# nii-yamagishilab/NELE-GAN

Measured on AMD Instinct MI355X. Metric: utterances/sec per GAN_epoch step (G+D+metric loss), higher is better.
Workload: dtype bf16

## Files before the change

### nele_gan_amd/csrc/haspi.hip

```cpp
#include "common.h"
#include <type_traits>
#include <cstdlib>

#define HP_NCH 32
#define HP_FS 24000.0
#define HP_LEVEL 65.0
#define HP_NBASIS 6
#define HP_NMOD 10
#define HP_NWIN 32769
#define HP_NTAB 512
#define HP_SPACE 9
#define HP_NFILT 52
#define HP_NHALF 26

typedef float hp_env_t;

struct HaspiWs {
    double* win;
    float* r24;
    double* mid;
    hp_env_t* ctl;
    hp_env_t* env;
    double* bw;
    double* loss;
    double* ssp;
// ... 8 lines not shown
    int fmul;
    double* benv;
    double* bkt;
    int* shift;
    double* lp;
    int* act;
    int* grank;
    int* gcnt;
    double* cpsum;
    double* cmean;
    int ngb;
    int* info;
    double* cep;
    double* cm;
    double* xf;
    double* cpart;
    const int* lens;
    float* cphi;
    double* sse;
    int fs_in;
    int n24, nsub;
    int nlp, lp_raw;
    int n24p;
};

__device__ __forceinline__ int hp_len(const HaspiWs& ws, int b, int L) { return ws.lens ? min(ws.lens[b], L) : L; }
__host__ __device__ static inline int hp_n24_of(int L, int fs_in) { return fs_in == 24000 ? L : (int)ceil((double)L * (24000.0 / (double)fs_in)); }
__host__ __device__ static inline int hp_nres_of(int L, int fs_in) { return fs_in == 24000 ? L : (int)((double)L * (24000.0 / (double)fs_in)); }
__device__ __forceinline__ int hp_n24(const HaspiWs& ws, int b) {
    if (!ws.lens) return ws.n24;
    return min(ws.n24, hp_n24_of(ws.lens[b], ws.fs_in));
}
__device__ __forceinline__ int hp_nsub(const HaspiWs& ws, int b) { return (hp_n24(ws, b) + HP_SPACE - 1) / HP_SPACE; }
__device__ __forceinline__ int hp_row(int idx, int sig0, int nsig) { return nsig == 2 ? idx : 2 * idx + sig0; }

__device__ __forceinline__ int hp_lp_di(const HaspiWs& ws, int b, int ch) {
    if (!ws.lp_raw) return 0;
    const int sh = ws.shift[(size_t)b * HP_NCH + ch];
    const int ul = (((26 - sh) % 9) + 9) % 9;
    return (ul + sh - 26) / 9;
}
__device__ __forceinline__ double hp_lp_at(const double* __restrict__ lpb, int i, int ch, int di) {
    const int g = i - di;
    return g >= 0 ? lpb[(size_t)g * HP_NCH + ch] : 0.0;
}

// ... 457 lines not shown
        }
        if (part == 0) {
#pragma unroll
            for (int u = 0; u < HP_CH; ++u) out[(size_t)(n0 + u) * HP_NCH] = (hp_env_t)eo[u];
        }
    }
    return ss;
}

#define GS_RC 16
#define GS_LC 1536
#define GS_MAXC 160
__device__ __forceinline__ void hp_rotate(double& cold, double& sold, double cn, double sn) {
    const double arg = fma(sold, sn, cold * cn);
    sold = fma(sold, cn, -(cold * sn));
    cold = arg;
}
__device__ __forceinline__ void hp_gt_step(const GtCoef& c, double x, double y, double& r0, double& r1, double& r2, double& r3) {
    r0 = fma(c.a1, x + y, r1);
    r1 = fma(c.a5, x, fma(c.a2, y, r2));
    r2 = fma(c.a3, y, r3);
    r3 = c.a4 * y;
}
__global__ __launch_bounds__(128) void haspi_pmat_kernel(HaspiWs ws, int lc, int signal, int sig0, int nsig) {
    const int ch = threadIdx.x & 31, k = threadIdx.x >> 5;
    const int row = signal ? hp_row(blockIdx.x, sig0, nsig) : 0;
    const double BW = signal ? ws.bw[(size_t)row * HP_NCH + ch] : hp_bw1(ch);
    const GtCoef c = hp_gt(BW, hp_cfreq(ch));
    double r0 = (k == 0), r1 = (k == 1), r2 = (k == 2), r3 = (k == 3);
    for (int n = 0; n < lc; ++n) {
        const double yr = r0;
        r0 = c.a1 * yr + r1;
        r1 = c.a2 * yr + r2;
        r2 = c.a3 * yr + r3;
        r3 = c.a4 * yr;
    }
    double* P = ws.pmat + ((size_t)(signal ? 1 + row : 0) * HP_NCH + ch) * 16;
    P[0 * 4 + k] = r0; P[1 * 4 + k] = r1; P[2 * 4 + k] = r2; P[3 * 4 + k] = r3;
}

template <bool SIGNAL>
__global__ __launch_bounds__(64) void haspi_bank_prefix_kernel(HaspiWs ws, int sig0, int nsig) {
    const int row = hp_row(blockIdx.x, sig0, nsig), lane = threadIdx.x, ch = lane & 31;
    const int n24 = hp_n24(ws, row >> 1);
    const int nch = ((n24 + GS_RC - 1) / GS_RC * GS_RC + ws.lc - 1) / ws.lc;
    const double* P = ws.pmat + ((size_t)(SIGNAL ? 1 + row : 0) * HP_NCH + ch) * 16;
    double Pm[16];
#pragma unroll
    for (int q = 0; q < 16; ++q) Pm[q] = P[q];
    double* est = ws.est + (size_t)row * ws.nchunk * 256 + lane;
    double r0 = 0, r1 = 0, r2 = 0, r3 = 0;
    constexpr int G = 8;
    for (int j0 = 0; j0 < nch; j0 += G) {
        double e[G][4];
#pragma unroll
        for (int g = 0; g < G; ++g) {
            const int j = min(j0 + g, nch - 1);
#pragma unroll
            for (int q = 0; q < 4; ++q) e[g][q] = est[(size_t)j * 256 + 64 * q];
        }
#pragma unroll
        for (int g = 0; g < G; ++g) {
            if (j0 + g < nch) {
                double* o = est + (size_t)(j0 + g) * 256;
                o[0] = r0; o[64] = r1; o[128] = r2; o[192] = r3;
                const double t0 = ((Pm[0] * r0 + Pm[1] * r1) + (Pm[2] * r2 + Pm[3] * r3)) + e[g][0];
                const double t1 = ((Pm[4] * r0 + Pm[5] * r1) + (Pm[6] * r2 + Pm[7] * r3)) + e[g][1];
                const double t2 = ((Pm[8] * r0 + Pm[9] * r1) + (Pm[10] * r2 + Pm[11] * r3)) + e[g][2];
                const double t3 = ((Pm[12] * r0 + Pm[13] * r1) + (Pm[14] * r2 + Pm[15] * r3)) + e[g][3];
// ... 10 lines not shown
__device__ __forceinline__ float hp_exp2f(float x) { return __builtin_amdgcn_exp2f(x); }
struct IhcC { double R2, R12C1, R23C2, a11, a12, a21, a22, denom, R1inv, c10, c11, c12, c20, c21, c22; };
__device__ __forceinline__ IhcC hp_ihc_consts() {
    const double delta = 2.0;
    const double tau1 = 0.001 * 2, tau2 = 0.001 * 60;
    const double T = 1 / HP_FS;
    const double R1 = 1 / delta, R2 = 0.5 * (1 - R1), R3 = R2;
    const double C1 = tau1 * (R1 + R2) / (R1 * R2);
    const double C2 = tau2 / ((R1 + R2) * R3);
    IhcC k;
    k.a11 = R1 + R2 + R1 * R2 * (C1 / T); k.a12 = -R1; k.a21 = -R3; k.a22 = R2 + R3 + R2 * R3 * (C2 / T);
    k.denom = 1.0 / (k.a11 * k.a22 - k.a21 * k.a12);
    k.R1inv = 1.0 / R1; k.R12C1 = R1 * R2 * (C1 / T); k.R23C2 = R2 * R3 * (C2 / T); k.R2 = R2;
    k.c10 = k.denom * k.a22 * k.R2;  k.c11 = k.denom * k.a22 * k.R12C1;  k.c12 = -k.denom * k.a12 * k.R23C2;
    k.c20 = -k.denom * k.a21 * k.R2; k.c21 = -k.denom * k.a21 * k.R12C1; k.c22 = k.denom * k.a11 * k.R23C2;
    return k;
}
__device__ __forceinline__ void hp_ihc_step(const IhcC& k, double V0, double& V1, double& V2) {
    const double t1 = fma(k.c12, V2, fma(k.c11, V1, V0 * k.c10));
    const double t2 = fma(k.c22, V2, fma(k.c21, V1, V0 * k.c20));
    V1 = t1; V2 = t2;
}

template <bool SIGNAL, bool PASS2, bool BM = false, bool GAIN = false>
__global__ __launch_bounds__(64) void haspi_bank_scan_kernel(HaspiWs ws, int sig0) {
    const int b = blockIdx.z, sig = sig0 + blockIdx.y, lane = threadIdx.x, ch = lane & 31;
    const int chunk = 2 * blockIdx.x + (lane >> 5);
    const int row = 2 * b + sig, lc = ws.lc;
    const int n24 = hp_n24(ws, b);
    const int n0 = chunk * lc, n1 = min(n0 + lc, (n24 + GS_RC - 1) / GS_RC * GS_RC);
    if (n0 >= n1) return;
    const double cf = hp_cfreq(ch);
    const GtCoef c = hp_gt(SIGNAL ? ws.bw[(size_t)row * HP_NCH + ch] : hp_bw1(ch), cf);
    const double tpt = 2.0 * M_PI / HP_FS;
    const double cn = cos(tpt * cf), sn = sin(tpt * cf);
    double* est = ws.est + ((size_t)row * ws.nchunk + chunk) * 256 + ch;
    double r0 = 0, r1 = 0, r2 = 0, r3 = 0, i0 = 0, i1 = 0, i2 = 0, i3 = 0;
    if (PASS2) {
        r0 = est[0]; r1 = est[64]; r2 = est[128]; r3 = est[192];
        i0 = est[32]; i1 = est[96]; i2 = est[160]; i3 = est[224];
    }
    double cold, sold;
    {
        const double ang = tpt * cf * (double)(n0 - 1);
        cold = cos(ang);
        sold = -sin(ang);
    }
// ... 8 lines not shown
    const double gb0 = 0.095107983402496, ga1 = -0.809784033195007;
    const IhcC ik = hp_ihc_consts();
    float knee = 30.0f, attn = 0.f;
    if (GAIN) {
        const HpLoss ls = hp_loss(ws, sig, ch);
        slope = (float)(1.0 - (1.0 / ls.CR));
        knee = (float)ls.lowknee; attn = (float)ls.attnOHC;
        c_off = (float)(HP_LEVEL + 20.0 * log10(hp_gt(hp_bw1(ch), cf).gain));
        s_off = (float)(HP_LEVEL - ls.attnIHC + 20.0 * log10(c.gain));
        for (int n = max(0, n0 - GL_W); n < n0; n += GL_U) {
            float gc[GL_U];
#pragma unroll
            for (int u = 0; u < GL_U; ++u) gc[u] = ctl[(size_t)(n + u) * HP_NCH];
#pragma unroll
            for (int u = 0; u < GL_U; ++u) {
                float le = c_off + TEN_LOG10_2 * hp_log2f(gc[u]);
                le = fminf(fmaxf(le, knee), 100.0f);
                const double gx = (double)hp_exp2f((-attn - (le - knee) * slope) * LOG2_10_OVER_20);
                const double y = gb0 * gx + gz;
                gz = gb0 * gx - ga1 * y;
            }
        }
    }
    for (int nb = n0; nb < n1; nb += GS_RC) {
        double xc[GS_RC];
        const hp_env_t* ctl_nb = ctl + (size_t)nb * HP_NCH;
        hp_env_t* out_nb = out + (size_t)nb * HP_NCH;
        float* cph_nb = BM ? cph + (size_t)nb * HP_NCH : nullptr;
#pragma unroll
        for (int u = 0; u < GS_RC / 2; ++u) {
            const double2 v = *reinterpret_cast<const double2*>(xin + nb + 2 * u);
            xc[2 * u] = v.x; xc[2 * u + 1] = v.y;
        }
        float eo[GS_RC], co[BM ? GS_RC : 1];
        auto bank = [&](auto tail_tag) {
            constexpr bool TAIL = decltype(tail_tag)::value;
#pragma unroll
            for (int u = 0; u < GS_RC; ++u) {
                hp_rotate(cold, sold, cn, sn);
                const double xr = xc[u] * cold, xi = xc[u] * sold;
                const double yr = xr + r0, yi = xi + i0;
                hp_gt_step(c, xr, yr, r0, r1, r2, r3);
                hp_gt_step(c, xi, yi, i0, i1, i2, i3);
                if (PASS2) {
                    const double e2 = yr * yr + yi * yi;
                    eo[u] = (float)e2;
                    if (!SIGNAL || BM) ss += (!TAIL || nb + u < n24) ? e2 : 0.0;
                    if (BM) co[u] = e2 > 0.0 ? (float)((yr * cold + yi * sold) / sqrt(e2)) : 0.f;
                }
            }
        };
        if (PASS2 && (!SIGNAL || BM) && nb + GS_RC > n24) bank(std::true_type{}); else bank(std::false_type{});
        if (GAIN) {
            float gc[GS_RC];
#pragma unroll
            for (int u = 0; u < GS_RC; ++u) gc[u] = ctl_nb[u * HP_NCH];
#pragma unroll
            for (int u = 0; u < GS_RC; ++u) {
                float le = c_off + TEN_LOG10_2 * hp_log2f(gc[u]);
                le = fminf(fmaxf(le, knee), 100.0f);
                const double gx = (double)hp_exp2f((-attn - (le - knee) * slope) * LOG2_10_OVER_20);
                const double yl = gb0 * gx + gz;
                gz = gb0 * gx - ga1 * yl;
                const float g = (float)yl;
                float y = s_off + TEN_LOG10_2 * hp_log2f(g * g * eo[u]);
                y = y > 0.0f ? y : 0.0f;
                eo[u] = y;
                hp_ihc_step(ik, (double)y, V1, V2);
            }
        }
        if (PASS2) {
#pragma unroll
            for (int u = 0; u < GS_RC; ++u) out_nb[u * HP_NCH] = eo[u];
            if (BM) {
#pragma unroll
                for (int u = 0; u < GS_RC; ++u) cph_nb[u * HP_NCH] = co[u];
            }
        }
    }
    if (!PASS2) {
        est[0] = r0; est[64] = r1; est[128] = r2; est[192] = r3;
        est[32] = i0; est[96] = i1; est[160] = i2; est[224] = i3;
    } else if (!SIGNAL) {
        ws.ssp[((size_t)row * ws.nchunk + chunk) * HP_NCH + ch] = ss;
    } else if (BM) {
        ws.sse[((size_t)row * ws.nchunk + chunk) * HP_NCH + ch] = ss;
    }
    if (GAIN) {
        const int ncg = (ws.n24p + ws.lcg - 1) / ws.lcg;
        double* ihe = ws.ihe + ((size_t)row * ncg + chunk) * 64 + ch;
        ihe[0] = V1; ihe[32] = V2;
    }
}

template <bool SIGNAL>
__global__ __launch_bounds__(512) void haspi_bank_tail_kernel(HaspiWs ws, int sig0, int nsig, int full, int nrows) {
    __shared__ double stage[2][64][GS_RC + 1];
    __shared__ int wred[8];
    const int id = (int)blockIdx.x, slot = id >> 3, cgrp = slot & 3, rest = slot >> 2;
    const int ncg = (ws.nchunk + 63) / 64;
    const int ridx = (rest / ncg) * 8 + (id & 7);
    if (ridx >= nrows) return;
    const int row = hp_row(ridx, sig0, nsig), b = row >> 1;
    const int tid = threadIdx.x, lane = tid & 63, wv = tid >> 6, ch = 8 * cgrp + wv;
    const int c0 = 64 * (rest % ncg), chunk = c0 + lane, lc = ws.lc;
    const int n24 = hp_n24(ws, b), nend = (n24 + GS_RC - 1) / GS_RC * GS_RC;
    const int n0 = chunk * lc, n1 = min(n0 + lc, nend);
    const bool live = n0 < n1;
    const double cf = hp_cfreq(ch);
    const double BW = SIGNAL ? ws.bw[(size_t)row * HP_NCH + ch] : hp_bw1(ch);
    const GtCoef c = hp_gt(BW, cf);
    const double tpt = 2.0 * M_PI / HP_FS;
    int W;
    {
        const double la = BW * tpt * (24.7 + cf / 9.26449) * 1.019;
        const double npk = fmax(3.0 / la, 1.0);
        const double peak = 3.0 * log(npk) - la * npk;
        double nn = 60.0 / la;
// ... 3 lines not shown
        if (full == 1) W = lc;
        if (full == 2) W = GS_RC;
    }
    if (lane == 0) wred[wv] = W;
    __syncthreads();
    int Wmax = wred[0];
#pragma unroll
    for (int q = 1; q < 8; ++q) Wmax = max(Wmax, wred[q]);
    const double cn = cos(tpt * cf), sn = sin(tpt * cf);
    double cold, sold;
    {
        const double ang = tpt * cf * (double)(n1 - W - 1);
        cold = cos(ang);
        sold = -sin(ang);
    }
    const double* xin = ws.mid + (size_t)row * ws.n24p;
    const int cc = tid >> 3, part = tid & 7;
    const int cn0 = (c0 + cc) * lc, cn1 = min(cn0 + lc, nend);
    const double* psrc = xin + (cn1 - Wmax + 2 * part);
    const int pfirst = (cn0 < cn1) ? cn0 - (cn1 - Wmax + 2 * part) : 0x7fffffff;
    double2 pv = (0 >= pfirst) ? *reinterpret_cast<const double2*>(psrc) : make_double2(0.0, 0.0);
    double r0 = 0, r1 = 0, r2 = 0, r3 = 0, i0 = 0, i1 = 0, i2 = 0, i3 = 0;
    const int tjoin = Wmax - W;
    for (int t = 0, it = 0; t < Wmax; t += GS_RC, ++it) {
        double (*st)[GS_RC + 1] = stage[it & 1];
        st[cc][2 * part] = pv.x; st[cc][2 * part + 1] = pv.y;
        __syncthreads();
        if (t + GS_RC < Wmax) pv = (t + GS_RC >= pfirst) ? *reinterpret_cast<const double2*>(psrc + t + GS_RC) : make_double2(0.0, 0.0);
        if (t >= tjoin) {
            double xc[GS_RC];
#pragma unroll
            for (int u = 0; u < GS_RC; ++u) xc[u] = st[lane][u];
#pragma unroll
            for (int u = 0; u < GS_RC; ++u) {
                hp_rotate(cold, sold, cn, sn);
                const double xr = xc[u] * cold, xi = xc[u] * sold;
                const double yr = xr + r0, yi = xi + i0;
                hp_gt_step(c, xr, yr, r0, r1, r2, r3);
                hp_gt_step(c, xi, yi, i0, i1, i2, i3);
            }
        }
    }
    if (live) {
        double* est = ws.est + ((size_t)row * ws.nchunk + chunk) * 256 + ch;
        est[0] = r0; est[64] = r1; est[128] = r2; est[192] = r3;
        est[32] = i0; est[96] = i1; est[160] = i2; est[224] = i3;
    }
}
__global__ void haspi_bw_kernel(HaspiWs ws, int sig0, int nsig) {
    const int row = hp_row(blockIdx.x, sig0, nsig), ch = threadIdx.x;
    const double bw1 = hp_bw1(ch);
    const GtCoef cc = hp_gt(bw1, hp_cfreq(ch));
    const int n24 = hp_n24(ws, row >> 1);
    const int nch = (n24 + ws.lc - 1) / ws.lc;
    double ss = 0.0;
    for (int c = 0; c < nch; ++c) ss += ws.ssp[((size_t)row * ws.nchunk + c) * HP_NCH + ch];
    ss *= cc.gain * cc.gain;
    const double cdB = 20.0 * log10(sqrt(ss / (double)n24)) + HP_LEVEL;
    const double bwmin = hp_loss(ws, row & 1, ch).BWmin;
    double BW;
    if (cdB < 50.0) BW = bwmin;
    else if (cdB > 100.0) BW = bw1;
    else BW = bwmin + ((cdB - 50.0) / 50.0) * (bw1 - bwmin);
    ws.bw[(size_t)row * HP_NCH + ch] = BW;
// ... 924 lines not shown
    TAKE(est, double, (size_t)B * 2 * nchunk * 256);
    TAKE(pmat, double, (size_t)(1 + B * 2) * HP_NCH * 16);
    TAKE(ihe, double, (size_t)B * 2 * ncg * 64);
    TAKE(pihc, double, 4);
    TAKE(rsp, double, (size_t)B * 2 * RS_MAXC);
    TAKE(rinfo, float, (size_t)B * 2 * 4);
    TAKE(benv, double, 64);
    TAKE(bkt, double, 10 * 616);
    TAKE(shift, int, (size_t)B * HP_NCH);
    TAKE(lp, double, (size_t)B * 2 * (nsub + 4) * HP_NCH);
    const int ngb = (nsub + CP_F - 1) / CP_F;
    TAKE(act, int, (size_t)B * nsub);
    TAKE(grank, int, (size_t)B * nsub);
    TAKE(gcnt, int, (size_t)B * ngb);
    TAKE(cpsum, double, (size_t)B * 2 * ngb * HP_NBASIS);
    TAKE(cmean, double, (size_t)B * 2 * HP_NBASIS);
    TAKE(info, int, (size_t)B * 2);
    TAKE(cep, double, (size_t)B * 2 * HP_NBASIS * nsub);
    TAKE(cm, double, (size_t)B * HP_NBASIS * HP_NMOD);
    TAKE(xf, double, (size_t)B * 64 * nsub);
    TAKE(cpart, double, (size_t)B * MS_MAXC * 64 * 5);
#undef TAKE
    if (w) { w->n24 = n24; w->nsub = nsub; w->n24p = n24p; w->fs_in = fs_in; w->lens = nullptr; w->nchunk = nchunk; w->lc = lc; w->ngb = ngb;
             w->cphi = nullptr; w->sse = nullptr; w->lcg = GL_N; w->fmul = 1; w->nlp = nsub + 4; w->lp_raw = 0; }
    return o;
}

extern "C" long long nele_metric_haspi_workspace_bytes(int B, int L, int fs_in) { return (long long)haspi_layout(B, L, fs_in, nullptr, nullptr); }

extern "C" int nele_metric_haspi_clean_sections(int B, int L, int fs_in, long long* out, int max_sections) {
    NELE_CHECK_ARG(B > 0 && out && max_sections >= 16, "nele_metric_haspi_clean_sections: bad arguments (16 sections)");
    NELE_CHECK_ARG(fs_in >= 1000 && fs_in <= 24000 && L >= 2400, "nele_metric_haspi_clean_sections: bad signal geometry");
    HaspiWs w;
    char* base = reinterpret_cast<char*>((uintptr_t)1 << 20);
    haspi_layout(B, L, fs_in, &w, base);
    int k = 0;
    auto put = [&](const void* p, long long stride, long long bytes) {
        out[3 * k] = (long long)(reinterpret_cast<const char*>(p) - base); out[3 * k + 1] = stride; out[3 * k + 2] = bytes; ++k;
    };
    const size_t ns = (size_t)w.nsub;
    put(w.win, 0, sizeof(double) * (HP_NWIN_AL + RS3_TAB));
    put(w.pmat, 0, sizeof(double) * HP_NCH * 16);
    put(w.pihc, 0, sizeof(double) * 4);
    put(w.benv, 0, sizeof(double) * 64);
    put(w.bkt, 0, sizeof(double) * 10 * 616);
    put(w.bw, sizeof(double) * 2 * HP_NCH, sizeof(double) * 2 * HP_NCH);
    put(w.rinfo, sizeof(float) * 2 * 4, sizeof(float) * 2 * 4);
    put(w.shift, sizeof(int) * HP_NCH, sizeof(int) * HP_NCH);
    put(w.act, sizeof(int) * ns, sizeof(int) * ns);
    put(w.grank, sizeof(int) * ns, sizeof(int) * ns);
    put(w.gcnt, sizeof(int) * (size_t)w.ngb, sizeof(int) * (size_t)w.ngb);
    put(w.cpsum, sizeof(double) * 2 * (size_t)w.ngb * HP_NBASIS, sizeof(double) * (size_t)w.ngb * HP_NBASIS);
    put(w.cmean, sizeof(double) * 2 * HP_NBASIS, sizeof(double) * 2 * HP_NBASIS);
    put(w.info, sizeof(int) * 2, sizeof(int) * 2);
    put(w.cep, sizeof(double) * 2 * HP_NBASIS * ns, sizeof(double) * HP_NBASIS * ns);
    put(w.xf, sizeof(double) * 64 * ns, sizeof(double) * 64 * ns);
    return k;
}

extern "C" int nele_metric_haspi_nsub(int L, int fs_in) {
    const int n24 = hp_n24_of(L, fs_in);
    return (n24 + HP_SPACE - 1) / HP_SPACE;
}

struct HaspiFlags { int par_iir, fused_gain, fir9; };
static const HaspiFlags& haspi_flags() {
    static HaspiFlags f = [] {
        HaspiFlags v;
        v.par_iir = NELE_SWITCH_INT("NELE_HASPI_PAR_IIR", 1) != 0;
        v.fused_gain = NELE_SWITCH_INT("NELE_HASPI_FUSED_GAIN", 1) != 0;
        v.fir9 = NELE_SWITCH_INT("NELE_HASPI_FIR9", 1) != 0;
        return v;
    }();
    return f;
}
static int haspi_lp_raw() { const HaspiFlags& f = haspi_flags(); return f.par_iir && f.fused_gain && f.fir9; }

static void haspi_build_window(const HaspiWs& ws, hipStream_t s) {
    hipLaunchKernelGGL(haspi_win_kernel, dim3((HP_NWIN + 255) / 256), dim3(256), 0, s, ws.win);
    hipLaunchKernelGGL(haspi_rs_taps_kernel, dim3(1), dim3(256), 0, s, ws.win);
}

static void haspi_chain(const float* x, const float* y, int B, int L, int fs_in, const HaspiWs& ws_in, int sig0, int nsig, hipStream_t s,
                        bool quality = false) {
    const int rows = B * nsig;
    HaspiWs ws = ws_in;
    const HaspiFlags& fl = haspi_flags();
    int par_iir = fl.par_iir, fused_gain = fl.fused_gain;
    if (quality) par_iir = fused_gain = 1;
    const bool in_bank = par_iir && fused_gain && !quality;
    ws.lcg = in_bank ? ws.lc : GL_N;
    ws.fmul = 1;
    hipLaunchKernelGGL(haspi_rms_kernel, dim3(B, nsig), dim3(256), 0, s, x, y, L, fs_in, ws, sig0);
    if (fs_in != 24000) {
        const int rs3 = NELE_SWITCH_INT("NELE_HASPI_RS3", 1);
        if (fs_in == 16000 && rs3)
            hipLaunchKernelGGL(haspi_resample3_kernel, dim3((ws.n24 + RS_CH - 1) / RS_CH, nsig, B), dim3(256), 0, s, x, y, L, ws, sig0);
        else
            hipLaunchKernelGGL(haspi_resample_kernel, dim3((ws.n24 + RS_CH - 1) / RS_CH, nsig, B), dim3(256), 0, s, x, y, L, ws, sig0);
        hipLaunchKernelGGL(haspi_resample_gain_kernel, dim3(rows), dim3(64), 0, s, ws, sig0, nsig);
    }
    if (par_iir) hipLaunchKernelGGL(haspi_midear_par_kernel, dim3(((ws.n24p + ME_N - 1) / ME_N + 63) / 64, rows), dim3(64), 0, s, ws, sig0, nsig);
    else { NELE_AB_ONLY(hipLaunchKernelGGL(haspi_midear_kernel, dim3(B), dim3(64), 0, s, ws, sig0, nsig);) }
    if (par_iir) {
        if (sig0 == 0) hipLaunchKernelGGL(haspi_pmat_kernel, dim3(1), dim3(128), 0, s, ws, ws.lc, 0, 0, 1);
        const int tail1 = NELE_SWITCH_INT("NELE_HASPI_TAIL1", 1);
        if (tail1) hipLaunchKernelGGL(haspi_bank_tail_kernel<false>, dim3(8 * 4 * ((ws.nchunk + 63) / 64) * ((rows + 7) / 8)), dim3(512), 0, s, ws, sig0, nsig, tail1 >= 2 ? tail1 - 1 : 0, rows);
        else { NELE_AB_ONLY(hipLaunchKernelGGL((haspi_bank_scan_kernel<false, false>), dim3((ws.nchunk + 1) / 2, nsig, B), dim3(64), 0, s, ws, sig0);) }
        hipLaunchKernelGGL(haspi_bank_prefix_kernel<false>, dim3(rows), dim3(64), 0, s, ws, sig0, nsig);
        hipLaunchKernelGGL((haspi_bank_scan_kernel<false, true>), dim3((ws.nchunk + 1) / 2, nsig, B), dim3(64), 0, s, ws, sig0);
        hipLaunchKernelGGL(haspi_bw_kernel, dim3(rows), dim3(32), 0, s, ws, sig0, nsig);
        hipLaunchKernelGGL(haspi_pmat_kernel, dim3(rows), dim3(128), 0, s, ws, ws.lc, 1, sig0, nsig);
        if (tail1) hipLaunchKernelGGL(haspi_bank_tail_kernel<true>, dim3(8 * 4 * ((ws.nchunk + 63) / 64) * ((rows + 7) / 8)), dim3(512), 0, s, ws, sig0, nsig, tail1 >= 2 ? tail1 - 1 : 0, rows);
        else { NELE_AB_ONLY(hipLaunchKernelGGL((haspi_bank_scan_kernel<true, false>), dim3((ws.nchunk + 1) / 2, nsig, B), dim3(64), 0, s, ws, sig0);) }
        hipLaunchKernelGGL(haspi_bank_prefix_kernel<true>, dim3(rows), dim3(64), 0, s, ws, sig0, nsig);
        if (quality) hipLaunchKernelGGL((haspi_bank_scan_kernel<true, true, true>), dim3((ws.nchunk + 1) / 2, nsig, B), dim3(64), 0, s, ws, sig0);
        else if (in_bank)
            NELE_PROF("haspi_bank_gain_kernel", s,
                      hipLaunchKernelGGL((haspi_bank_scan_kernel<true, true, false, true>), dim3((ws.nchunk + 1) / 2, nsig, B), dim3(64), 0, s, ws, sig0));
        else { NELE_AB_ONLY(hipLaunchKernelGGL((haspi_bank_scan_kernel<true, true>), dim3((ws.nchunk + 1) / 2, nsig, B), dim3(64), 0, s, ws, sig0);) }
    } else {
        NELE_AB_ONLY(hipLaunchKernelGGL(haspi_control_kernel, dim3(nsig, B), dim3(64), 0, s, ws, sig0);
                     hipLaunchKernelGGL(haspi_signal_kernel, dim3(nsig, B), dim3(64), 0, s, ws, sig0);)
    }
    if (sig0 == 0) hipLaunchKernelGGL(haspi_shift_kernel, dim3(B), dim3(64), 0, s, ws);
    if (fused_gain && par_iir) {
        if (!in_bank)
            NELE_PROF("haspi_gain_lp_sl_kernel", s,
                      hipLaunchKernelGGL(haspi_gain_lp_sl_kernel, dim3((ws.n24p + 8 * GL_N - 1) / (8 * GL_N), rows), dim3(256), 0, s, ws, sig0, nsig));
        hipLaunchKernelGGL(haspi_ihc_prefix_kernel, dim3(rows), dim3(32), 0, s, ws, sig0, nsig);
        if (quality) return;
        const dim3 fgrid((ws.n24p + 4 * ws.lcg * ws.fmul - 1) / (4 * ws.lcg * ws.fmul), rows);
        if (ws.lp_raw) hipLaunchKernelGGL(haspi_ihc_fir9_kernel, fgrid, dim3(128), 0, s, ws, sig0, nsig);
        else { NELE_AB_ONLY(hipLaunchKernelGGL(haspi_ihc_fir_kernel, fgrid, dim3(128), 0, s, ws, sig0, nsig);) }
        return;
    }
#ifdef NELE_AB
    else {
        if (fused_gain) {
            hipLaunchKernelGGL(haspi_gain_lp_sl_kernel, dim3((ws.n24p + 8 * GL_N - 1) / (8 * GL_N), rows), dim3(256), 0, s, ws, sig0, nsig);
        } else {
            const size_t per_row = (size_t)ws.n24p * HP_NCH;
            const unsigned bx = (unsigned)((per_row + 255) / 256 < 256 ? (per_row + 255) / 256 : 256);
            hipLaunchKernelGGL(haspi_gain_kernel, dim3(bx, rows), dim3(256), 0, s, ws, per_row, sig0, nsig);
            hipLaunchKernelGGL(haspi_gainlp_kernel, dim3((rows + 1) / 2), dim3(64), 0, s, ws, sig0, nsig, rows);
            hipLaunchKernelGGL(haspi_sl_kernel, dim3(bx, rows), dim3(256), 0, s, ws, per_row, sig0, nsig);
        }
        hipLaunchKernelGGL(haspi_ihc_kernel, dim3((rows + 1) / 2), dim3(64), 0, s, ws, sig0, nsig, rows);
    }
    hipLaunchKernelGGL(haspi_envfilt_kernel, dim3((ws.nsub + EF_SUB - 1) / EF_SUB, B, nsig), dim3(256), 0, s, ws, sig0);
#endif
}

static int haspi_hl_table(const double* hl6, int itype, HpHL* out) {
    if (itype != 0 && itype != 2)
        return nele_set_error(NELE_ERR_UNSUPPORTED, "HASPI ear model: itype %d (NAL-R) is not implemented by the reference either (eb_NALR raises)", itype);
    for (int k = 0; k < 6; ++k) {
        const double v = hl6 ? hl6[k] : 0.0;
        out->y[k] = v;
        out->x[k] = itype == 0 ? 0.0 : v;
    }
    return NELE_OK;
}

static int haspi_var_impl(const float* x, const float* y, const int* lengths, int B, int L, int fs_in, const double* dither, const double* hl6, int itype,
                          void* workspace, long long workspace_bytes, float* raw, float* mapped, int* info_out, int phase, void* stream);

extern "C" int nele_metric_haspi_var(const float* x, const float* y, const int* lengths, int B, int L, int fs_in, const double* dither,
                                     void* workspace, long long workspace_bytes, float* raw, float* mapped, int* info_out, int phase,
                                     void* stream) {
    return haspi_var_impl(x, y, lengths, B, L, fs_in, dither, nullptr, 0, workspace, workspace_bytes, raw, mapped, info_out, phase, stream);
}

extern "C" int nele_metric_haspi_var_hl(const float* x, const float* y, const int* lengths, int B, int L, int fs_in, const double* dither,
// ... 3 lines not shown
}

static int haspi_var_impl(const float* x, const float* y, const int* lengths, int B, int L, int fs_in, const double* dither, const double* hl6, int itype,
                          void* workspace, long long workspace_bytes, float* raw, float* mapped, int* info_out, int phase, void* stream) {
    NELE_CHECK_ARG(workspace && B > 0 && (phase == 0 || phase == 3 || phase == 4), "nele_metric_haspi: bad arguments");
    HpHL hl;
    { const int st_ = haspi_hl_table(hl6, itype, &hl); if (st_) return st_; }
    NELE_CHECK_ARG((x || phase == 4) && (y || phase == 3) && (raw || mapped || phase == 3), "nele_metric_haspi: missing signal / output for phase %d", phase);
    NELE_CHECK_ARG(fs_in >= 1000 && fs_in <= 24000, "nele_metric_haspi: fs must be in [1000, 24000] Hz (got %d; the reference has no downsampler)", fs_in);
    if (L < 2400) return nele_set_error(NELE_ERR_SIGNAL, "nele_metric_haspi: L=%d too short", L);
    if (workspace_bytes < nele_metric_haspi_workspace_bytes(B, L, fs_in))
        return nele_set_error(NELE_ERR_WORKSPACE, "nele_metric_haspi: workspace too small");
    HaspiWs ws;
    haspi_layout(B, L, fs_in, &ws, (char*)workspace);
    ws.lens = lengths;
    ws.lp_raw = haspi_lp_raw();
    hipStream_t s = as_stream(stream);
    hipLaunchKernelGGL(haspi_loss_kernel, dim3(1), dim3(64), 0, s, ws, hl);
    const int cep_serial = NELE_SWITCH_INT("NELE_HASPI_CEP_SERIAL", 1);
    const int mod_direct = NELE_SWITCH_INT("NELE_HASPI_MOD_DIRECT", 0);
    NELE_CHECK_ARG((ws.nsub + MS_TC - 1) / MS_TC <= MS_MAXC, "nele_metric_haspi: signal too long (%d sub-sampled frames)", ws.nsub);
    if (phase == 0 || phase == 3) {
        if (fs_in != 24000) haspi_build_window(ws, s);
        haspi_chain(x, y, B, L, fs_in, ws, 0, 1, s);
        if (cep_serial) {
            hipLaunchKernelGGL(haspi_cep_kernel, dim3(B), dim3(256), 0, s, ws, dither, 0.1, 1, 0, 1);
        } else {
            NELE_AB_ONLY(hipLaunchKernelGGL(haspi_gate_kernel, dim3(ws.ngb, B), dim3(CP_F), 0, s, ws);
                         hipLaunchKernelGGL(haspi_gate_scan_kernel, dim3(B), dim3(64), 0, s, ws);
                         hipLaunchKernelGGL(haspi_cepstra_kernel, dim3(ws.ngb, B, 1), dim3(CP_F), 0, s, ws, dither, 0.1, 0);
                         hipLaunchKernelGGL(haspi_cepmean_kernel, dim3(B, 1), dim3(64), 0, s, ws, 0);)
        }
        if (mod_direct) { NELE_AB_ONLY(hipLaunchKernelGGL(haspi_mod_direct_kernel<0>, dim3(HP_NMOD, HP_NBASIS - 1, B), dim3(256), 0, s, ws);) }
        else hipLaunchKernelGGL(haspi_mod_slide_kernel<0>, dim3((ws.nsub + MS_TC - 1) / MS_TC, B), dim3(64), 0, s, ws);
    }
    if (phase == 0 || phase == 4) {
        haspi_chain(x, y, B, L, fs_in, ws, 1, 1, s);
        if (cep_serial) {
            hipLaunchKernelGGL(haspi_cep_kernel, dim3(B), dim3(256), 0, s, ws, dither, 0.1, 0, 1, 1);
        } else {
            NELE_AB_ONLY(hipLaunchKernelGGL(haspi_cepstra_kernel, dim3(ws.ngb, B, 1), dim3(CP_F), 0, s, ws, dither, 0.1, 1);
                         hipLaunchKernelGGL(haspi_cepmean_kernel, dim3(B, 1), dim3(64), 0, s, ws, 1);)
        }
        if (mod_direct) { NELE_AB_ONLY(hipLaunchKernelGGL(haspi_mod_direct_kernel<1>, dim3(HP_NMOD, HP_NBASIS - 1, B), dim3(256), 0, s, ws);) }
        else {
            hipLaunchKernelGGL(haspi_mod_slide_kernel<1>, dim3((ws.nsub + MS_TC - 1) / MS_TC, B), dim3(64), 0, s, ws);
            hipLaunchKernelGGL(haspi_modcorr_kernel, dim3(B), dim3(64), 0, s, ws);
        }
        hipLaunchKernelGGL(haspi_final_kernel, dim3((B + 63) / 64), dim3(64), 0, s, ws, raw, mapped, B);
    }
    if (info_out) (void)hipMemcpyAsync(info_out, ws.info, sizeof(int) * 2 * (size_t)B, hipMemcpyDeviceToDevice, s);
    NELE_CHECK_LAUNCH("nele_metric_haspi");
    return NELE_OK;
}

extern "C" int nele_metric_haspi(const float* x, const float* y, int B, int L, int fs_in, const double* dither, void* workspace,
                                 long long workspace_bytes, float* raw, float* mapped, int* info_out, void* stream) {
    NELE_CHECK_ARG(x && y && (raw || mapped), "nele_metric_haspi: bad arguments");
    return nele_metric_haspi_var(x, y, nullptr, B, L, fs_in, dither, workspace, workspace_bytes, raw, mapped, info_out, 0, stream);
}
// ... 23 lines not shown
```

### nele_gan_amd/csrc/haspi_quality.h

```cpp
#define HQ_NWIN 384
#define HQ_NHALF 192
#define HQ_MAXLAG 24
#define HQ_NOUT 12
#define HQ_MAXBINS 2048

struct QualWs {
    double* sm;
    double* cov;
    double* msx;
    double* msy;
    double* corr;
    double* segl;
    int* qinfo;
    int nseg;
    unsigned long long seed;
    int noise;
    const long long* ids;
};

__device__ __forceinline__ int hq_nseg(int n24) { return 1 + n24 / HQ_NWIN + (n24 - HQ_NHALF) / HQ_NWIN; }
__device__ __forceinline__ double hq_win(int k) { return 0.5 - 0.5 * cospi(2.0 * (double)k / (double)(HQ_NWIN - 1)); }

__device__ __forceinline__ unsigned long long hq_mix(unsigned long long z) {
    z += 0x9E3779B97F4A7C15ull;
// ... 489 lines not shown
extern "C" int nele_metric_haspi_quality_hl(const float* x, const float* y, const int* lengths, int B, int L, int fs_in, int noise,
                                            unsigned long long seed, double alpha, const double* hl6_host, int itype, void* workspace,
                                            long long workspace_bytes, double* out, int* info_out, void* stream) {
    return haspi_quality_impl(x, y, lengths, B, L, fs_in, noise, seed, alpha, hl6_host, itype, workspace, workspace_bytes, out, info_out, stream);
}

static int haspi_quality_impl(const float* x, const float* y, const int* lengths, int B, int L, int fs_in, int noise, unsigned long long seed, double alpha,
                              const double* hl6, int itype, void* workspace, long long workspace_bytes, double* out, int* info_out, void* stream) {
    NELE_CHECK_ARG(x && y && out && workspace && B > 0, "nele_metric_haspi_quality: bad arguments");
    HpHL hl;
    { const int st_ = haspi_hl_table(hl6, itype, &hl); if (st_) return st_; }
    NELE_CHECK_ARG(fs_in >= 1000 && fs_in <= 24000, "nele_metric_haspi_quality: fs must be in [1000, 24000] Hz (got %d; the reference has no downsampler)", fs_in);
    if (L < 2400) return nele_set_error(NELE_ERR_SIGNAL, "nele_metric_haspi_quality: L=%d too short", L);
    if (workspace_bytes < nele_metric_haspi_quality_workspace_bytes(B, L, fs_in))
        return nele_set_error(NELE_ERR_WORKSPACE, "nele_metric_haspi_quality: workspace too small");
    HaspiWs ws;
    QualWs q;
    quality_layout(B, L, fs_in, &ws, &q, (char*)workspace);
    ws.lens = lengths;
    q.seed = seed; q.noise = noise ? 1 : 0; q.ids = nullptr;
    hipStream_t s = as_stream(stream);
    hipLaunchKernelGGL(haspi_loss_kernel, dim3(1), dim3(64), 0, s, ws, hl);
    if (fs_in != 24000) haspi_build_window(ws, s);
    haspi_chain(x, y, B, L, fs_in, ws, 0, 2, s, true);
    const int rows = 2 * B;
    hipLaunchKernelGGL(hq_ihc_bm_kernel, dim3(((ws.n24p + GL_N - 1) / GL_N + 7) / 8, rows), dim3(256), 0, s, ws, q, 0, 2);
    hipLaunchKernelGGL(hq_corr_kernel, dim3(1), dim3(128), 0, s, q);
    hipLaunchKernelGGL(hq_segment_kernel<0>, dim3(q.nseg, 4, B), dim3(128), 0, s, ws, q);
    hipLaunchKernelGGL(hq_loud_kernel, dim3((q.nseg + 63) / 64, B), dim3(64), 0, s, ws, q);
    hipLaunchKernelGGL(hq_final_kernel<true>, dim3(B), dim3(256), 0, s, ws, q, alpha, out);
    if (info_out) (void)hipMemcpyAsync(info_out, q.qinfo, sizeof(int) * 4 * (size_t)B, hipMemcpyDeviceToDevice, s);
    NELE_CHECK_LAUNCH("nele_metric_haspi_quality");
    return NELE_OK;
}

extern "C" long long nele_metric_hasqi_workspace_bytes(int B, int L, int fs_in) {
    return (long long)quality_layout(B, L, fs_in, nullptr, nullptr, nullptr);
}

extern "C" int nele_metric_hasqi_clean_sections(int B, int L, int fs_in, long long* out, int max_sections) {
    NELE_CHECK_ARG(B > 0 && out && max_sections >= 12, "nele_metric_hasqi_clean_sections: bad arguments (12 sections)");
    NELE_CHECK_ARG(fs_in >= 1000 && fs_in <= 24000 && L >= 2400, "nele_metric_hasqi_clean_sections: bad signal geometry");
    HaspiWs w;
    QualWs q;
    char* base = reinterpret_cast<char*>((uintptr_t)1 << 20);
    quality_layout(B, L, fs_in, &w, &q, base);
    int k = 0;
// ... 21 lines not shown
                                     double* out, int* info_out, int phase, void* stream) {
    NELE_CHECK_ARG(workspace && B > 0 && (phase == 0 || phase == 3 || phase == 4), "nele_metric_hasqi_var: bad arguments");
    NELE_CHECK_ARG((x || phase == 4) && (y || phase == 3) && (out || phase == 3), "nele_metric_hasqi_var: missing signal / output for phase %d", phase);
    NELE_CHECK_ARG(noise >= 0 && noise <= 2 && (noise != 2 || utt_ids), "nele_metric_hasqi_var: noise must be 0, 1 or 2 (2 needs utt_ids)");
    HpHL hl;
    { const int st_ = haspi_hl_table(hl6_host, 2, &hl); if (st_) return st_; }
    NELE_CHECK_ARG(fs_in >= 1000 && fs_in <= 24000, "nele_metric_hasqi_var: fs must be in [1000, 24000] Hz (got %d; the reference has no downsampler)", fs_in);
    if (L < 2400) return nele_set_error(NELE_ERR_SIGNAL, "nele_metric_hasqi_var: L=%d too short", L);
    if (workspace_bytes < nele_metric_hasqi_workspace_bytes(B, L, fs_in))
        return nele_set_error(NELE_ERR_WORKSPACE, "nele_metric_hasqi_var: workspace too small");
    HaspiWs ws;
    QualWs q;
    quality_layout(B, L, fs_in, &ws, &q, (char*)workspace);
    ws.lens = lengths;
    q.seed = seed; q.noise = noise; q.ids = utt_ids;
    hipStream_t s = as_stream(stream);
    const dim3 igrid(((ws.n24p + GL_N - 1) / GL_N + 7) / 8, B), sgrid(q.nseg, 4, B), lgrid((q.nseg + 63) / 64, B);
    hipLaunchKernelGGL(haspi_loss_kernel, dim3(1), dim3(64), 0, s, ws, hl);
    if (phase != 4) {
        if (fs_in != 24000) haspi_build_window(ws, s);
        hipLaunchKernelGGL(hq_corr_kernel, dim3(1), dim3(128), 0, s, q);
    }
    if (phase == 0) {
        haspi_chain(x, y, B, L, fs_in, ws, 0, 2, s, true);
        hipLaunchKernelGGL(hq_ihc_bm_kernel, dim3(igrid.x, 2 * B), dim3(256), 0, s, ws, q, 0, 2);
        hipLaunchKernelGGL(hq_segment_kernel<0>, sgrid, dim3(128), 0, s, ws, q);
        hipLaunchKernelGGL(hq_loud_kernel, lgrid, dim3(64), 0, s, ws, q);
    } else if (phase == 3) {
        haspi_chain(x, y, B, L, fs_in, ws, 0, 1, s, true);
        hipLaunchKernelGGL(hq_ihc_bm_kernel, igrid, dim3(256), 0, s, ws, q, 0, 1);
        hipLaunchKernelGGL(hq_segment_kernel<1>, sgrid, dim3(128), 0, s, ws, q);
        hipLaunchKernelGGL(hq_loud_kernel, lgrid, dim3(64), 0, s, ws, q);
    } else {
        haspi_chain(x, y, B, L, fs_in, ws, 1, 1, s, true);
        hipLaunchKernelGGL(hq_ihc_bm_kernel, igrid, dim3(256), 0, s, ws, q, 1, 1);
        hipLaunchKernelGGL(hq_segment_kernel<2>, sgrid, dim3(128), 0, s, ws, q);
    }
    if (phase != 3) {
        hipLaunchKernelGGL((hq_final_kernel<false>), dim3(B), dim3(256), 0, s, ws, q, -1.0, out);
        if (info_out) (void)hipMemcpyAsync(info_out, q.qinfo, sizeof(int) * 4 * (size_t)B, hipMemcpyDeviceToDevice, s);
    }
    NELE_CHECK_LAUNCH("nele_metric_hasqi_var");
    return NELE_OK;
}
```

Baseline: 7546.

## Replace HASPI gammatone and IHC recurrences in chunk kernels with precomputed impulse-response tables

Precomputes per-channel impulse-response tables, one time per device and chunk length, for the reference gammatone filter and the IHC adaptation filter, along with the chunk transfer matrix. Chunk-local recurrences in the bank tail and gain scan kernels become independent FMAs against table entries instead of serial rotate-and-filter steps. The per-call pmat launch is dropped. This shortens the serial dependency chains but adds table loads. It also adds a one-time blocking build that must happen outside stream capture.

Result: no change. 7501 (-0.6%).

```diff
diff --git a/nele_gan_amd/csrc/haspi.hip b/nele_gan_amd/csrc/haspi.hip
--- a/nele_gan_amd/csrc/haspi.hip
+++ b/nele_gan_amd/csrc/haspi.hip
@@ -1,6 +1,8 @@
 #include "common.h"
 #include <type_traits>
 #include <cstdlib>
+#include <mutex>
+#include <vector>
 
 #define HP_NCH 32
 #define HP_FS 24000.0
@@ -55,6 +57,9 @@
     int n24, nsub;
     int nlp, lp_raw;
     int n24p;
+    const double* tihc;
+    const double* tctl;
+    const double* tpm;
 };
 
 __device__ __forceinline__ int hp_len(const HaspiWs& ws, int b, int L) { return ws.lens ? min(ws.lens[b], L) : L; }
@@ -558,11 +563,7 @@
     r2 = fma(c.a3, y, r3);
     r3 = c.a4 * y;
 }
-__global__ __launch_bounds__(128) void haspi_pmat_kernel(HaspiWs ws, int lc, int signal, int sig0, int nsig) {
-    const int ch = threadIdx.x & 31, k = threadIdx.x >> 5;
-    const int row = signal ? hp_row(blockIdx.x, sig0, nsig) : 0;
-    const double BW = signal ? ws.bw[(size_t)row * HP_NCH + ch] : hp_bw1(ch);
-    const GtCoef c = hp_gt(BW, hp_cfreq(ch));
+__device__ __forceinline__ void hp_pmat_col(const GtCoef& c, int lc, int k, double* __restrict__ P) {
     double r0 = (k == 0), r1 = (k == 1), r2 = (k == 2), r3 = (k == 3);
     for (int n = 0; n < lc; ++n) {
         const double yr = r0;
@@ -571,8 +572,13 @@
         r2 = c.a3 * yr + r3;
         r3 = c.a4 * yr;
     }
-    double* P = ws.pmat + ((size_t)(signal ? 1 + row : 0) * HP_NCH + ch) * 16;
     P[0 * 4 + k] = r0; P[1 * 4 + k] = r1; P[2 * 4 + k] = r2; P[3 * 4 + k] = r3;
+}
+__global__ __launch_bounds__(128) void haspi_pmat_kernel(HaspiWs ws, int lc, int signal, int sig0, int nsig) {
+    const int ch = threadIdx.x & 31, k = threadIdx.x >> 5;
+    const int row = signal ? hp_row(blockIdx.x, sig0, nsig) : 0;
+    const double BW = signal ? ws.bw[(size_t)row * HP_NCH + ch] : hp_bw1(ch);
+    hp_pmat_col(hp_gt(BW, hp_cfreq(ch)), lc, k, ws.pmat + ((size_t)(signal ? 1 + row : 0) * HP_NCH + ch) * 16);
 }
 
 template <bool SIGNAL>
@@ -580,7 +586,7 @@
     const int row = hp_row(blockIdx.x, sig0, nsig), lane = threadIdx.x, ch = lane & 31;
     const int n24 = hp_n24(ws, row >> 1);
     const int nch = ((n24 + GS_RC - 1) / GS_RC * GS_RC + ws.lc - 1) / ws.lc;
-    const double* P = ws.pmat + ((size_t)(SIGNAL ? 1 + row : 0) * HP_NCH + ch) * 16;
+    const double* P = SIGNAL ? ws.pmat + ((size_t)(1 + row) * HP_NCH + ch) * 16 : ws.tpm + (size_t)ch * 16;
     double Pm[16];
 #pragma unroll
     for (int q = 0; q < 16; ++q) Pm[q] = P[q];
@@ -637,7 +643,46 @@
     V1 = t1; V2 = t2;
 }
 
-template <bool SIGNAL, bool PASS2, bool BM = false, bool GAIN = false>
+__global__ __launch_bounds__(256) void haspi_tables_kernel(double* __restrict__ tihc, double* __restrict__ tctl, double* __restrict__ tpm, int lc) {
+    const int ch = blockIdx.x, tid = threadIdx.x;
+    if (ch == HP_NCH) {
+        if (tid != 0) return;
+        const IhcC ik = hp_ihc_consts();
+        double V1 = 0.0, V2 = 0.0;
+        for (int k = 0; k < lc; ++k) {
+            hp_ihc_step(ik, k == 0 ? 1.0 : 0.0, V1, V2);
+            tihc[2 * k] = V1; tihc[2 * k + 1] = V2;
+        }
+        return;
+    }
+    const double cf = hp_cfreq(ch);
+    const GtCoef c = hp_gt(hp_bw1(ch), cf);
+    double* T = tctl + (size_t)ch * lc * 8;
+    if (tid == 0) {
+        double r0 = 0, r1 = 0, r2 = 0, r3 = 0;
+        for (int k = 0; k < lc; ++k) {
+            const double x = k == 0 ? 1.0 : 0.0;
+            hp_gt_step(c, x, x + r0, r0, r1, r2, r3);
+            T[8 * k] = r0; T[8 * k + 1] = r1; T[8 * k + 2] = r2; T[8 * k + 3] = r3;
+        }
+    } else if (tid <= 4) {
+        hp_pmat_col(c, lc, tid - 1, tpm + (size_t)ch * 16);
+    }
+    __threadfence_block();
+    __syncthreads();
+    const double w = 2.0 * M_PI / HP_FS * cf;
+    for (int k = tid; k < lc; k += 256) {
+        const double ck = cos(w * (double)k), sk = sin(w * (double)k);
+#pragma unroll
+        for (int q = 0; q < 4; ++q) {
+            const double h = T[8 * k + q];
+            T[8 * k + q] = h * ck;
+            T[8 * k + 4 + q] = h * sk;
+        }
+    }
+}
+
+template <bool SIGNAL, bool PASS2, bool BM = false, bool GAIN = false, bool TAB = false>
 __global__ __launch_bounds__(64) void haspi_bank_scan_kernel(HaspiWs ws, int sig0) {
     const int b = blockIdx.z, sig = sig0 + blockIdx.y, lane = threadIdx.x, ch = lane & 31;
     const int chunk = 2 * blockIdx.x + (lane >> 5);
@@ -692,8 +737,10 @@
             }
         }
     }
-    for (int nb = n0; nb < n1; nb += GS_RC) {
+    for (int off = 0; n0 + off < n1; off += GS_RC) {
+        const int nb = n0 + off;
         double xc[GS_RC];
+        const double* __restrict__ wtab = TAB ? ws.tihc + 2 * (size_t)__builtin_amdgcn_readfirstlane(lc - GS_RC - off) : nullptr;
         const hp_env_t* ctl_nb = ctl + (size_t)nb * HP_NCH;
         hp_env_t* out_nb = out + (size_t)nb * HP_NCH;
         float* cph_nb = BM ? cph + (size_t)nb * HP_NCH : nullptr;
@@ -736,7 +783,12 @@
                 float y = s_off + TEN_LOG10_2 * hp_log2f(g * g * eo[u]);
                 y = y > 0.0f ? y : 0.0f;
                 eo[u] = y;
-                hp_ihc_step(ik, (double)y, V1, V2);
+                if (TAB) {
+                    V1 = fma(wtab[2 * (GS_RC - 1 - u)], (double)y, V1);
+                    V2 = fma(wtab[2 * (GS_RC - 1 - u) + 1], (double)y, V2);
+                } else {
+                    hp_ihc_step(ik, (double)y, V1, V2);
+                }
             }
         }
         if (PASS2) {
@@ -763,7 +815,7 @@
     }
 }
 
-template <bool SIGNAL>
+template <bool SIGNAL, bool TAB = false>
 __global__ __launch_bounds__(512) void haspi_bank_tail_kernel(HaspiWs ws, int sig0, int nsig, int full, int nrows) {
     __shared__ double stage[2][64][GS_RC + 1];
     __shared__ int wred[8];
@@ -813,6 +865,7 @@
     double2 pv = (0 >= pfirst) ? *reinterpret_cast<const double2*>(psrc) : make_double2(0.0, 0.0);
     double r0 = 0, r1 = 0, r2 = 0, r3 = 0, i0 = 0, i1 = 0, i2 = 0, i3 = 0;
     const int tjoin = Wmax - W;
+    const double* __restrict__ wch = TAB ? ws.tctl + (size_t)__builtin_amdgcn_readfirstlane(ch) * lc * 8 : nullptr;
     for (int t = 0, it = 0; t < Wmax; t += GS_RC, ++it) {
         double (*st)[GS_RC + 1] = stage[it & 1];
         st[cc][2 * part] = pv.x; st[cc][2 * part + 1] = pv.y;
@@ -822,15 +875,32 @@
             double xc[GS_RC];
 #pragma unroll
             for (int u = 0; u < GS_RC; ++u) xc[u] = st[lane][u];
-#pragma unroll
-            for (int u = 0; u < GS_RC; ++u) {
-                hp_rotate(cold, sold, cn, sn);
-                const double xr = xc[u] * cold, xi = xc[u] * sold;
-                const double yr = xr + r0, yi = xi + i0;
-                hp_gt_step(c, xr, yr, r0, r1, r2, r3);
-                hp_gt_step(c, xi, yi, i0, i1, i2, i3);
+            if (TAB) {
+                const double* __restrict__ wg = wch + 8 * (size_t)__builtin_amdgcn_readfirstlane(W - GS_RC - (t - tjoin));
+#pragma unroll
+                for (int u = 0; u < GS_RC; ++u) {
+                    const double* __restrict__ w8 = wg + 8 * (GS_RC - 1 - u);
+                    r0 = fma(w8[0], xc[u], r0); r1 = fma(w8[1], xc[u], r1); r2 = fma(w8[2], xc[u], r2); r3 = fma(w8[3], xc[u], r3);
+                    i0 = fma(w8[4], xc[u], i0); i1 = fma(w8[5], xc[u], i1); i2 = fma(w8[6], xc[u], i2); i3 = fma(w8[7], xc[u], i3);
+                }
+            } else {
+#pragma unroll
+                for (int u = 0; u < GS_RC; ++u) {
+                    hp_rotate(cold, sold, cn, sn);
+                    const double xr = xc[u] * cold, xi = xc[u] * sold;
+                    const double yr = xr + r0, yi = xi + i0;
+                    hp_gt_step(c, xr, yr, r0, r1, r2, r3);
+                    hp_gt_step(c, xi, yi, i0, i1, i2, i3);
+                }
             }
         }
+    }
+    if (TAB) {
+        const double ang = tpt * cf * (double)(n1 - 1);
+        const double cm = cos(ang), sm = sin(ang);
+        const double a0 = r0, a1 = r1, a2 = r2, a3 = r3;
+        r0 = fma(cm, a0, sm * i0); r1 = fma(cm, a1, sm * i1); r2 = fma(cm, a2, sm * i2); r3 = fma(cm, a3, sm * i3);
+        i0 = fma(cm, i0, -(sm * a0)); i1 = fma(cm, i1, -(sm * a1)); i2 = fma(cm, i2, -(sm * a2)); i3 = fma(cm, i3, -(sm * a3));
     }
     if (live) {
         double* est = ws.est + ((size_t)row * ws.nchunk + chunk) * 256 + ch;
@@ -1801,7 +1871,7 @@
     TAKE(cpart, double, (size_t)B * MS_MAXC * 64 * 5);
 #undef TAKE
     if (w) { w->n24 = n24; w->nsub = nsub; w->n24p = n24p; w->fs_in = fs_in; w->lens = nullptr; w->nchunk = nchunk; w->lc = lc; w->ngb = ngb;
-             w->cphi = nullptr; w->sse = nullptr; w->lcg = GL_N; w->fmul = 1; w->nlp = nsub + 4; w->lp_raw = 0; }
+             w->cphi = nullptr; w->sse = nullptr; w->tihc = w->tctl = w->tpm = nullptr; w->lcg = GL_N; w->fmul = 1; w->nlp = nsub + 4; w->lp_raw = 0; }
     return o;
 }
 
@@ -1842,12 +1912,13 @@
     return (n24 + HP_SPACE - 1) / HP_SPACE;
 }
 
-struct HaspiFlags { int par_iir, fused_gain, fir9; };
+struct HaspiFlags { int par_iir, fused_gain, fir9, tables; };
 static const HaspiFlags& haspi_flags() {
     static HaspiFlags f = [] {
         HaspiFlags v;
         v.par_iir = NELE_SWITCH_INT("NELE_HASPI_PAR_IIR", 1) != 0;
         v.fused_gain = NELE_SWITCH_INT("NELE_HASPI_FUSED_GAIN", 1) != 0;
+        v.tables = NELE_SWITCH_INT("NELE_HASPI_TABLES", 1) != 0;
         v.fir9 = NELE_SWITCH_INT("NELE_HASPI_FIR9", 1) != 0;
         return v;
     }();
@@ -1860,7 +1931,35 @@
     hipLaunchKernelGGL(haspi_rs_taps_kernel, dim3(1), dim3(256), 0, s, ws.win);
 }
 
-static void haspi_chain(const float* x, const float* y, int B, int L, int fs_in, const HaspiWs& ws_in, int sig0, int nsig, hipStream_t s,
+struct HaspiTables { int dev, lc; double* base; };
+static int haspi_tables(int lc, hipStream_t s, HaspiWs* ws) {
+    static std::mutex mu;
+    static std::vector<HaspiTables> built;
+    int dev = 0;
+    if (hipGetDevice(&dev) != hipSuccess) return nele_set_error(NELE_ERR_HIP, "HASPI tables: hipGetDevice failed");
+    const size_t n_ihc = 2 * (size_t)lc, n_pm = (size_t)HP_NCH * 16, n_ctl = (size_t)HP_NCH * lc * 8;
+    std::lock_guard<std::mutex> lock(mu);
+    double* base = nullptr;
+    for (const HaspiTables& t : built)
+        if (t.dev == dev && t.lc == lc) base = t.base;
+    if (!base) {
+        hipStreamCaptureStatus cap = hipStreamCaptureStatusNone;
+        if (hipStreamIsCapturing(s, &cap) != hipSuccess || cap != hipStreamCaptureStatusNone)
+            return nele_set_error(NELE_ERR_HIP, "HASPI tables for chunk length %d are not built yet: make one call outside the stream capture first", lc);
+        if (hipMalloc(reinterpret_cast<void**>(&base), sizeof(double) * (n_ihc + n_pm + n_ctl)) != hipSuccess)
+            return nele_set_error(NELE_ERR_HIP, "HASPI tables: hipMalloc of %zu bytes failed", sizeof(double) * (n_ihc + n_pm + n_ctl));
+        hipLaunchKernelGGL(haspi_tables_kernel, dim3(HP_NCH + 1), dim3(256), 0, s, base, base + n_ihc + n_pm, base + n_ihc, lc);
+        if (hipGetLastError() != hipSuccess || hipStreamSynchronize(s) != hipSuccess) {
+            (void)hipFree(base);
+            return nele_set_error(NELE_ERR_HIP, "HASPI tables: building them failed");
+        }
+        built.push_back({dev, lc, base});
+    }
+    ws->tihc = base; ws->tpm = base + n_ihc; ws->tctl = base + n_ihc + n_pm;
+    return NELE_OK;
+}
+
+static int haspi_chain(const float* x, const float* y, int B, int L, int fs_in, const HaspiWs& ws_in, int sig0, int nsig, hipStream_t s,
                         bool quality = false) {
     const int rows = B * nsig;
     HaspiWs ws = ws_in;
@@ -1870,6 +1969,9 @@
     const bool in_bank = par_iir && fused_gain && !quality;
     ws.lcg = in_bank ? ws.lc : GL_N;
     ws.fmul = 1;
+    const bool tables = par_iir && fl.tables;
+    if (tables) { const int st_ = haspi_tables(ws.lc, s, &ws); if (st_) return st_; }
+    else ws.tpm = ws.pmat;
     hipLaunchKernelGGL(haspi_rms_kernel, dim3(B, nsig), dim3(256), 0, s, x, y, L, fs_in, ws, sig0);
     if (fs_in != 24000) {
         const int rs3 = NELE_SWITCH_INT("NELE_HASPI_RS3", 1);
@@ -1882,9 +1984,10 @@
     if (par_iir) hipLaunchKernelGGL(haspi_midear_par_kernel, dim3(((ws.n24p + ME_N - 1) / ME_N + 63) / 64, rows), dim3(64), 0, s, ws, sig0, nsig);
     else { NELE_AB_ONLY(hipLaunchKernelGGL(haspi_midear_kernel, dim3(B), dim3(64), 0, s, ws, sig0, nsig);) }
     if (par_iir) {
-        if (sig0 == 0) hipLaunchKernelGGL(haspi_pmat_kernel, dim3(1), dim3(128), 0, s, ws, ws.lc, 0, 0, 1);
+        if (!tables && sig0 == 0) { NELE_AB_ONLY(hipLaunchKernelGGL(haspi_pmat_kernel, dim3(1), dim3(128), 0, s, ws, ws.lc, 0, 0, 1);) }
         const int tail1 = NELE_SWITCH_INT("NELE_HASPI_TAIL1", 1);
-        if (tail1) hipLaunchKernelGGL(haspi_bank_tail_kernel<false>, dim3(8 * 4 * ((ws.nchunk + 63) / 64) * ((rows + 7) / 8)), dim3(512), 0, s, ws, sig0, nsig, tail1 >= 2 ? tail1 - 1 : 0, rows);
+        if (tail1 && tables) hipLaunchKernelGGL((haspi_bank_tail_kernel<false, true>), dim3(8 * 4 * ((ws.nchunk + 63) / 64) * ((rows + 7) / 8)), dim3(512), 0, s, ws, sig0, nsig, tail1 >= 2 ? tail1 - 1 : 0, rows);
+        else if (tail1) { NELE_AB_ONLY(hipLaunchKernelGGL(haspi_bank_tail_kernel<false>, dim3(8 * 4 * ((ws.nchunk + 63) / 64) * ((rows + 7) / 8)), dim3(512), 0, s, ws, sig0, nsig, tail1 >= 2 ? tail1 - 1 : 0, rows);) }
         else { NELE_AB_ONLY(hipLaunchKernelGGL((haspi_bank_scan_kernel<false, false>), dim3((ws.nchunk + 1) / 2, nsig, B), dim3(64), 0, s, ws, sig0);) }
         hipLaunchKernelGGL(haspi_bank_prefix_kernel<false>, dim3(rows), dim3(64), 0, s, ws, sig0, nsig);
         hipLaunchKernelGGL((haspi_bank_scan_kernel<false, true>), dim3((ws.nchunk + 1) / 2, nsig, B), dim3(64), 0, s, ws, sig0);
@@ -1894,9 +1997,13 @@
         else { NELE_AB_ONLY(hipLaunchKernelGGL((haspi_bank_scan_kernel<true, false>), dim3((ws.nchunk + 1) / 2, nsig, B), dim3(64), 0, s, ws, sig0);) }
         hipLaunchKernelGGL(haspi_bank_prefix_kernel<true>, dim3(rows), dim3(64), 0, s, ws, sig0, nsig);
         if (quality) hipLaunchKernelGGL((haspi_bank_scan_kernel<true, true, true>), dim3((ws.nchunk + 1) / 2, nsig, B), dim3(64), 0, s, ws, sig0);
-        else if (in_bank)
+        else if (in_bank && tables)
             NELE_PROF("haspi_bank_gain_kernel", s,
-                      hipLaunchKernelGGL((haspi_bank_scan_kernel<true, true, false, true>), dim3((ws.nchunk + 1) / 2, nsig, B), dim3(64), 0, s, ws, sig0));
+                      hipLaunchKernelGGL((haspi_bank_scan_kernel<true, true, false, true, true>), dim3((ws.nchunk + 1) / 2, nsig, B), dim3(64), 0, s, ws, sig0));
+        else if (in_bank) {
+            NELE_AB_ONLY(NELE_PROF("haspi_bank_gain_kernel", s,
+                      hipLaunchKernelGGL((haspi_bank_scan_kernel<true, true, false, true>), dim3((ws.nchunk + 1) / 2, nsig, B), dim3(64), 0, s, ws, sig0));)
+        }
         else { NELE_AB_ONLY(hipLaunchKernelGGL((haspi_bank_scan_kernel<true, true>), dim3((ws.nchunk + 1) / 2, nsig, B), dim3(64), 0, s, ws, sig0);) }
     } else {
         NELE_AB_ONLY(hipLaunchKernelGGL(haspi_control_kernel, dim3(nsig, B), dim3(64), 0, s, ws, sig0);
@@ -1908,11 +2015,11 @@
             NELE_PROF("haspi_gain_lp_sl_kernel", s,
                       hipLaunchKernelGGL(haspi_gain_lp_sl_kernel, dim3((ws.n24p + 8 * GL_N - 1) / (8 * GL_N), rows), dim3(256), 0, s, ws, sig0, nsig));
         hipLaunchKernelGGL(haspi_ihc_prefix_kernel, dim3(rows), dim3(32), 0, s, ws, sig0, nsig);
-        if (quality) return;
+        if (quality) return NELE_OK;
         const dim3 fgrid((ws.n24p + 4 * ws.lcg * ws.fmul - 1) / (4 * ws.lcg * ws.fmul), rows);
         if (ws.lp_raw) hipLaunchKernelGGL(haspi_ihc_fir9_kernel, fgrid, dim3(128), 0, s, ws, sig0, nsig);
         else { NELE_AB_ONLY(hipLaunchKernelGGL(haspi_ihc_fir_kernel, fgrid, dim3(128), 0, s, ws, sig0, nsig);) }
-        return;
+        return NELE_OK;
     }
 #ifdef NELE_AB
     else {
@@ -1929,6 +2036,7 @@
     }
     hipLaunchKernelGGL(haspi_envfilt_kernel, dim3((ws.nsub + EF_SUB - 1) / EF_SUB, B, nsig), dim3(256), 0, s, ws, sig0);
 #endif
+    return NELE_OK;
 }
 
 static int haspi_hl_table(const double* hl6, int itype, HpHL* out) {
@@ -1978,7 +2086,7 @@
     NELE_CHECK_ARG((ws.nsub + MS_TC - 1) / MS_TC <= MS_MAXC, "nele_metric_haspi: signal too long (%d sub-sampled frames)", ws.nsub);
     if (phase == 0 || phase == 3) {
         if (fs_in != 24000) haspi_build_window(ws, s);
-        haspi_chain(x, y, B, L, fs_in, ws, 0, 1, s);
+        { const int st_ = haspi_chain(x, y, B, L, fs_in, ws, 0, 1, s); if (st_) return st_; }
         if (cep_serial) {
             hipLaunchKernelGGL(haspi_cep_kernel, dim3(B), dim3(256), 0, s, ws, dither, 0.1, 1, 0, 1);
         } else {
@@ -1991,7 +2099,7 @@
         else hipLaunchKernelGGL(haspi_mod_slide_kernel<0>, dim3((ws.nsub + MS_TC - 1) / MS_TC, B), dim3(64), 0, s, ws);
     }
     if (phase == 0 || phase == 4) {
-        haspi_chain(x, y, B, L, fs_in, ws, 1, 1, s);
+        { const int st_ = haspi_chain(x, y, B, L, fs_in, ws, 1, 1, s); if (st_) return st_; }
         if (cep_serial) {
             hipLaunchKernelGGL(haspi_cep_kernel, dim3(B), dim3(256), 0, s, ws, dither, 0.1, 0, 1, 1);
         } else {
diff --git a/nele_gan_amd/csrc/haspi_quality.h b/nele_gan_amd/csrc/haspi_quality.h
--- a/nele_gan_amd/csrc/haspi_quality.h
+++ b/nele_gan_amd/csrc/haspi_quality.h
@@ -535,7 +535,7 @@
     hipStream_t s = as_stream(stream);
     hipLaunchKernelGGL(haspi_loss_kernel, dim3(1), dim3(64), 0, s, ws, hl);
     if (fs_in != 24000) haspi_build_window(ws, s);
-    haspi_chain(x, y, B, L, fs_in, ws, 0, 2, s, true);
+    { const int st_ = haspi_chain(x, y, B, L, fs_in, ws, 0, 2, s, true); if (st_) return st_; }
     const int rows = 2 * B;
     hipLaunchKernelGGL(hq_ihc_bm_kernel, dim3(((ws.n24p + GL_N - 1) / GL_N + 7) / 8, rows), dim3(256), 0, s, ws, q, 0, 2);
     hipLaunchKernelGGL(hq_corr_kernel, dim3(1), dim3(128), 0, s, q);
@@ -603,17 +603,17 @@
         hipLaunchKernelGGL(hq_corr_kernel, dim3(1), dim3(128), 0, s, q);
     }
     if (phase == 0) {
-        haspi_chain(x, y, B, L, fs_in, ws, 0, 2, s, true);
+        { const int st_ = haspi_chain(x, y, B, L, fs_in, ws, 0, 2, s, true); if (st_) return st_; }
         hipLaunchKernelGGL(hq_ihc_bm_kernel, dim3(igrid.x, 2 * B), dim3(256), 0, s, ws, q, 0, 2);
         hipLaunchKernelGGL(hq_segment_kernel<0>, sgrid, dim3(128), 0, s, ws, q);
         hipLaunchKernelGGL(hq_loud_kernel, lgrid, dim3(64), 0, s, ws, q);
     } else if (phase == 3) {
-        haspi_chain(x, y, B, L, fs_in, ws, 0, 1, s, true);
+        { const int st_ = haspi_chain(x, y, B, L, fs_in, ws, 0, 1, s, true); if (st_) return st_; }
         hipLaunchKernelGGL(hq_ihc_bm_kernel, igrid, dim3(256), 0, s, ws, q, 0, 1);
         hipLaunchKernelGGL(hq_segment_kernel<1>, sgrid, dim3(128), 0, s, ws, q);
         hipLaunchKernelGGL(hq_loud_kernel, lgrid, dim3(64), 0, s, ws, q);
     } else {
-        haspi_chain(x, y, B, L, fs_in, ws, 1, 1, s, true);
+        { const int st_ = haspi_chain(x, y, B, L, fs_in, ws, 1, 1, s, true); if (st_) return st_; }
         hipLaunchKernelGGL(hq_ihc_bm_kernel, igrid, dim3(256), 0, s, ws, q, 1, 1);
         hipLaunchKernelGGL(hq_segment_kernel<2>, sgrid, dim3(128), 0, s, ws, q);
     }
```
